# aurianer/DLA-Future

Measured on AMD Instinct MI355X. Metric: fp64 Cholesky TFlop/s, higher is better.
Workload: dtype f64; 1 GPU; cholesky_d N=65536 nb=1024 uplo=L; grid=1x1, rank_order=column-major, transport=none, work_copies=5

## Files before the change

### dla_future_amd/csrc/host/cholesky.cpp

```cpp
#include "device_matrix.hpp"
#include "launch_args.hpp"

#include <algorithm>
#include <cstdlib>
#include <cstring>
#include <vector>

namespace dlaf_mi355x {

static bool potrf_use_chain() {
  static const bool chain = [] {
    const char* e = std::getenv("DLAF_MI355X_POTRF");
    return e && std::strcmp(e, "chain") == 0;
  }();
  return chain;
}

template <class T>
void potrf_tile_coop(T* t, int ld, int kb, T* winv, int* info, int info_base, unsigned* sync, hipStream_t s,
                     bool sync_is_zero, bool count_strips) {
  launch_potrf_coop(t, ld, kb, winv, info, info_base, sync, s, sync_is_zero, count_strips);
}

template <class T>
void potrf_tile_chain(T* t, int ld, int kb, T* winv, int* info, int info_base, hipStream_t s) {
  constexpr int JB = kDiagBlock;
  for (int j0 = 0; j0 < kb; j0 += JB) {
    const int jb = std::min(JB, kb - j0);
    T* djj = t + j0 + (size_t) j0 * ld;
    T* wj = winv + (size_t) (j0 / JB) * JB * JB;
    launch_potrf_diag(djj, ld, jb, wj, info, info_base + j0, s);
    const int rem = kb - j0 - jb;
    if (rem <= 0)
      break;
    T* sub = t + (j0 + jb) + (size_t) j0 * ld;
    TrsmArgs<T> ta;
    ta.b = sub;
    ta.b_ts = 0;
    ta.ldb = ld;
    ta.il0 = 0;
    ta.il1 = 1;
    ta.pr = 1;
    ta.ri = 0;
    ta.nb = rem;
    ta.nt = 1;
    ta.last_rows = rem;
    ta.l = djj;
    ta.ldl = ld;
    ta.winv = wj;
    ta.n = jb;
    ta.info = info;
    launch_trsm(ta, s);
    UpdateArgs<T> ua;
    ua.c = t + (j0 + jb) + (size_t) (j0 + jb) * ld;
    ua.c_tsr = ua.c_tsc = 0;
    ua.ldc = ld;
    ua.a = sub;
    ua.a_ts = 0;
    ua.lda = ld;
    ua.b = sub;
    ua.b_ts = 0;
    ua.ldb = ld;
    ua.il0 = ua.jl0 = 0;
    ua.il1 = ua.jl1 = 1;
    ua.nb = rem;
    ua.K = jb;
    ua.pr = ua.pc = 1;
    ua.ri = ua.ci = 0;
    ua.nt = 1;
    ua.last_rows = rem;
    ua.info = info;
    launch_update(ua, s, 2);
  }
}

template <class T>
void potrf_tile(T* t, int ld, int kb, T* winv, int* info, int info_base, unsigned* sync, hipStream_t s) {
  if (!potrf_use_chain())
    potrf_tile_coop(t, ld, kb, winv, info, info_base, sync, s,  true,  true);
  else
    potrf_tile_chain(t, ld, kb, winv, info, info_base, s);
}

static long gcd_l(long a, long b) {
  while (b) {
    const long t = a % b;
    a = b;
    b = t;
  }
  return a;
}

template <class T>
int DeviceMatrix<T>::bcast_transposed_panel(Transport* tr, CommAxis ax_col, const T* a_base, long il_n, long jl_n,
                                            T* dst, hipStream_t s, int& period, long& ts2) {
  const size_t tile_bytes = tile_elems * sizeof(T);
  const long ncols = ltc - jl_n;
  const long g = gcd_l(rows.P, cols.P);
  period = (int) (rows.P / g);
  const long lstep = cols.P / g;
  const long cap = ncols > 0 ? (ncols + period - 1) / period : 0;
  ts2 = cap * (long) tile_elems;
  int issued = 0;
  tr->group_begin();
  for (long c = 0; c < period && c < ncols; ++c) {
    const long jl_first = jl_n + c;
    const long gj_first = cols.global_of(jl_first);
    const int root_r = rows.owner(gj_first);
    long cnt = (ncols - c + period - 1) / period;
    if (cols.global_of(jl_first + (cnt - 1) * period) == nt - 1)
      --cnt;
    if (cnt <= 0)
      continue;
    T* d = dst + c * ts2;
    if (rows.rank == root_r) {
      const T* src = a_base + (size_t) (rows.local_of(gj_first) - il_n) * tile_elems;
      DLAF_HIP_CHECK(hipMemcpy2DAsync(d, tile_bytes, src, (size_t) lstep * tile_bytes, tile_bytes, (size_t) cnt,
                                      hipMemcpyDeviceToDevice, s));
    }
    tr->bcast(ax_col, root_r, rows.rank, d, d, (size_t) cnt * tile_bytes, s);
    ++issued;
  }
  tr->group_end();
  return issued;
}

namespace {

enum class Schedule { Pairs, Sidecar, Early, Classic };

Schedule choose_schedule(bool dist, int nb, bool complex_type) {
  const char* e = std::getenv("DLAF_MI355X_SCHEDULE");
  if (e == nullptr) {
    if (dist)
      return Schedule::Early;
    if (nb % 16 == 0)
      return Schedule::Pairs;
    return !complex_type && nb <= 768 ? Schedule::Sidecar : Schedule::Classic;
  }
  if (std::strcmp(e, "early") == 0)
    return Schedule::Early;
  if (!dist && std::strcmp(e, "pairs") == 0)
    return Schedule::Pairs;
  if (!dist && std::strcmp(e, "sidecar") == 0)
    return Schedule::Sidecar;
  return Schedule::Classic;
}

constexpr long kSidecarSlots = 32;

template <class T>
struct PairRates {
  static constexpr bool dbl = sizeof(real_t<T>) == 8;
  static constexpr double r_bulk = dbl ? (TypeInfo<T>::is_complex ? 66e12 : 70e12) : 118e12;
  static constexpr double r_trsm_slot = (dbl ? 5e12 : 8e12) / 32.0;
  static constexpr double t_potrf_blk2 = 11.3e-6 * (TypeInfo<T>::is_complex ? 2.0 : 1.0);
};

template <class T>
struct Step {
  const T* a_base = nullptr;
  const T* b_base = nullptr;
  long b_ts = 0, il_n = 0, jl_n = 0;
  int b_period = 1;
  long b_ts2 = 0;
  const T* a2_base = nullptr;
  const T* b2_base = nullptr;
  int k1 = 0;
  int kb = 0;
  long rest0 = 0, split = 0;
  bool valid = false;

  static Step one_panel(int kb, long il_n, long jl_n, const T* a_base, size_t tile_elems) {
    Step st;
    st.valid = true;
    st.kb = kb;
    st.il_n = il_n;
    st.jl_n = jl_n;
    st.a_base = st.b_base = a_base;
    st.b_ts = (long) tile_elems;
    return st;
  }
  static Step two_panels(int k1, int k2, long n0, const T* a_base, const T* a2_base, size_t tile_elems) {
    Step st = one_panel(k1 + k2, n0, n0, a_base, tile_elems);
    st.k1 = k1;
    st.a2_base = st.b2_base = a2_base;
    return st;
  }
};

template <class T>
struct CholeskyIssue {
  using StepT = Step<T>;
  DeviceMatrix<T>& m;
  Transport* tr;
  const bool dist;
  const size_t tile_bytes;
  const CommAxis ax_row, ax_col;
  const hipStream_t s_main, s_panel, s_comm;
  long potrf_slots = 0, comm_slots = 0;
  long grid_reserve = 0;
  size_t next_update_slice = 0;

  explicit CholeskyIssue(DeviceMatrix<T>& mat)
      : m(mat), tr(checked_transport(*mat.grid)), dist(mat.grid->nranks > 1), tile_bytes(mat.tile_elems * sizeof(T)),
        ax_row(mat.transposed ? CommAxis::Col : CommAxis::Row),
        ax_col(mat.transposed ? CommAxis::Row : CommAxis::Col), s_main(mat.s_low), s_panel(mat.s_high),
        s_comm(mat.s_comm) {
    if (const char* e = std::getenv("DLAF_MI355X_POTRF_SLOTS"))
      potrf_slots = std::atol(e);
    else
      potrf_slots = potrf_use_chain() ? 0 : 2 * ((m.nb + kDiagBlock - 1) / kDiagBlock);
    if (const char* e = std::getenv("DLAF_MI355X_COMM_SLOTS"))
      comm_slots = std::atol(e);
    else
      comm_slots = (dist && tr->device_side()) ? 32 : 0;
    grid_reserve = potrf_slots + comm_slots;
  }

  StepT one_panel(long k, long il_n, long jl_n, const T* a_base) const {
    return StepT::one_panel(m.rows.tile_extent(k), il_n, jl_n, a_base, m.tile_elems);
  }

  void update_work(long il0, long il1, long j0, long j1, int kb, double& flops, double& bytes) const {
    flops = bytes = 0;
    const double cx = TypeInfo<T>::is_complex ? 4.0 : 1.0;
    for (long jl = j0; jl < j1; ++jl) {
      const long gj = m.cols.global_of(jl);
      const double nj = m.rows.tile_extent(gj);
      for (long il = std::max(il0, m.rows.next_local(gj)); il < il1; ++il) {
        const long gi = m.rows.global_of(il);
        const double mi = m.rows.tile_extent(gi);
        if (gi == gj) {
          flops += cx * mi * (mi + 1) * kb;
          bytes += (mi * kb + mi * mi) * sizeof(T);
        }
        else {
          flops += cx * 2.0 * mi * nj * kb;
          bytes += (mi * kb + nj * kb + 2.0 * mi * nj) * sizeof(T);
        }
      }
    }
  }

  double column_flops(const StepT& st, long jl) const {
    double f, by;
    update_work(std::max(st.il_n, m.rows.next_local(m.cols.global_of(jl))), m.ltr, jl, jl + 1, st.kb, f, by);
    return f;
  }

  void update(const StepT& st, long j0, long j1, hipStream_t s, int role, long reserve, long il_from = -1,
              long il_to = -1, int kind = -1) {
    if (!st.valid || j0 >= j1)
      return;
    const long il0 = std::max(std::max(st.il_n, il_from), m.rows.next_local(m.cols.global_of(j0)));
    const long il1 = il_to < 0 ? m.ltr : std::min(il_to, m.ltr);
    if (il0 >= il1)
      return;
    UpdateArgs<T> ua = update_args(m, il0, il1, j0, j1, st.a_base + (size_t) (il0 - st.il_n) * m.tile_elems, st.b_base,
                                   st.b_ts, st.kb, m.info);
    ua.b_period = st.b_period;
    ua.b_ts2 = st.b_ts2;
    ua.b_jl0 = (int) st.jl_n;
    if (st.k1 > 0) {
      ua.K1 = st.k1;
      ua.a2 = st.a2_base + (size_t) (il0 - st.il_n) * m.tile_elems;
      ua.b2 = st.b2_base;
    }
    double fl, by;
    update_work(il0, il1, j0, j1, st.kb, fl, by);
    const int pk = kind < 0 ? role : kind;
    m.prof_begin(pk, s);
    unsigned* cnt = m.coop_sync;
    bool zero = false;
    if (reserve > 0) {
      const size_t sl = std::min(next_update_slice, m.coop_sync_update_slices - 1);
      cnt = m.coop_sync + 16 * sl;
      zero = next_update_slice < m.coop_sync_update_slices - 1;
      ++next_update_slice;
    }
    static const bool exclusive = [] {
      const char* e = std::getenv("DLAF_MI355X_EXCLUSIVE_CUS");
      return e ? std::atoi(e) != 0 : true;
    }();
    if (reserve > 0 && exclusive)
      launch_update(ua, s, role, m.bulk_slots, cnt, zero, reserve);
    else
      launch_update(ua, s, role, reserve > 0 ? std::max<long>(8, m.bulk_slots - reserve) : 0, cnt, zero);
    DLAF_HIP_CHECK(hipGetLastError());
    m.prof_end(pk, s, fl, by);
  }

  void trsm(long il0, long il1, long klc, const T* Lkk, const T* Wkk, int kb, hipStream_t ts = nullptr) {
    if (ts == nullptr)
      ts = s_main;
    if (il0 >= il1)
      return;
    TrsmArgs<T> ta = panel_args<TrsmArgs<T>>(m, il0, il1, klc, Lkk, kb);
    ta.winv = Wkk;
    ta.info = m.info;
    ta.prio = (ts != s_main) ? 1 : 0;
    double fl = 0, by = 0;
    for (long il = il0; il < il1; ++il) {
      const double mi = m.rows.tile_extent(m.rows.global_of(il));
      fl += (TypeInfo<T>::is_complex ? 4.0 : 1.0) * (double) kb * kb * mi;
      by += (0.5 * kb * kb + 2.0 * mi * kb) * sizeof(T);
    }
    m.prof_begin(2, ts);
    launch_trsm(ta, ts);
    DLAF_HIP_CHECK(hipGetLastError());
    m.prof_end(2, ts, fl, by);
  }

  T* winv_of(long k) const { return m.winv + (size_t) (k & 1) * m.winv_elems(); }
  T* diag_ws_of(long k) const { return m.diag_ws + (size_t) (k & 1) * (m.tile_elems + m.winv_elems()); }
  void potrf(long k) {
    if (m.rows.rank != m.rows.owner(k) || m.cols.rank != m.cols.owner(k))
      return;
    const int kb = m.rows.tile_extent(k);
    const double cxf = TypeInfo<T>::is_complex ? 4.0 : 1.0;
    m.prof_begin(3, s_panel);
    potrf_tile(m.tile(m.rows.local_of(k), m.cols.local_of(k)), m.nb, kb, winv_of(k), m.info, (int) (k * m.nb),
               m.coop_sync + 16 * m.coop_sync_update_slices + m.coop_sync_potrf_words * (size_t) k, s_panel);
    DLAF_HIP_CHECK(hipGetLastError());
    m.prof_end(3, s_panel, cxf * (double) kb * kb * kb / 3.0, (double) kb * kb * sizeof(T));
  }

  void diag_bcast(long k, bool in_row, bool in_col, const T*& Lkk, const T*& Wkk) {
    Lkk = Wkk = nullptr;
    if (in_row && in_col) {
      Lkk = m.tile(m.rows.local_of(k), m.cols.local_of(k));
      Wkk = winv_of(k);
    }
    if (in_col && m.rows.P > 1) {
      T* ws = diag_ws_of(k);
      if (in_row) {
        DLAF_HIP_CHECK(hipMemcpyAsync(ws, Lkk, tile_bytes, hipMemcpyDeviceToDevice, s_panel));
        DLAF_HIP_CHECK(hipMemcpyAsync(ws + m.tile_elems, Wkk, m.winv_elems() * sizeof(T), hipMemcpyDeviceToDevice, s_panel));
      }
      DLAF_HIP_CHECK(hipEventRecord(m.ev_diag[k], s_panel));
      DLAF_HIP_CHECK(hipStreamWaitEvent(s_comm, m.ev_diag[k], 0));
      tr->bcast(ax_col, m.rows.owner(k), m.rows.rank, ws, ws, tile_bytes + m.winv_elems() * sizeof(T), s_comm);
      DLAF_HIP_CHECK(hipEventRecord(m.ev_diag[k], s_comm));
      Lkk = ws;
      Wkk = ws + m.tile_elems;
    }
    else {
      DLAF_HIP_CHECK(hipEventRecord(m.ev_diag[k], s_panel));
    }
  }

  void transposed_panel(StepT& cur, int buf) {
    if (m.rows.P > 1) {
      m.bcast_transposed_panel(tr, ax_col, cur.a_base, cur.il_n, cur.jl_n, m.panelT[buf], s_comm, cur.b_period,
                               cur.b_ts2);
      cur.b_base = m.panelT[buf];
      cur.b_ts = (long) m.tile_elems;
    }
    else {
      cur.b_base = cur.a_base + (m.cols.global_of(cur.jl_n) - cur.il_n) * (long) m.tile_elems;
      cur.b_ts = (long) m.tile_elems * m.cols.P;
    }
  }

  void join_last_diag(long k) {
    DLAF_HIP_CHECK(hipEventRecord(m.ev_diag[k], s_panel));
    DLAF_HIP_CHECK(hipStreamWaitEvent(s_main, m.ev_diag[k], 0));
  }

  void panel_done(long k, hipStream_t s) {
    DLAF_HIP_CHECK(hipEventRecord(m.ev_panel[k], s));
    m.panels_issued.store(k, std::memory_order_release);
  }

  long pair_slots(long k, double bulk_flops) const {
    using R = PairRates<T>;
    const long nb = m.nb, bulk_slots = m.bulk_slots;
    const double cxf = TypeInfo<T>::is_complex ? 4.0 : 1.0;
    const double below = (double) std::max<long>(0, m.n - (k + 1) * nb) + (double) std::max<long>(0, m.n - (k + 2) * nb);
    const double fl_t = cxf * (double) nb * nb * below;
    const double nblk = (double) nb / kDiagBlock;
    const double t_potrf = 2.0 * nblk * nblk * R::t_potrf_blk2;
    auto t_of = [&](long sl) {
      const double share = (double) sl / (double) bulk_slots;
      return std::max(bulk_flops / (R::r_bulk * (1.0 - share)), t_potrf + fl_t / (R::r_trsm_slot * (double) sl));
    };
    long best = kSidecarSlots;
    double best_t = t_of(best);
    if (bulk_flops / (R::r_bulk * (1.0 - (double) best / (double) bulk_slots)) >= best_t)
      return best;
    for (long cand : {48L, 64L, 96L, 128L, 192L, 256L}) {
      if (cand <= kSidecarSlots || cand * 2 > bulk_slots)
        continue;
      const double t = t_of(cand);
      if (t < best_t) {
        best_t = t;
        best = cand;
      }
    }
    return best;
  }

  bool u1_on_main(long k, long slots, double bulk_flops) const {
    using R = PairRates<T>;
    const long nb = m.nb;
    const double cxf = TypeInfo<T>::is_complex ? 4.0 : 1.0;
    const double below1 = (double) std::max<long>(0, m.n - (k + 1) * nb), below2 = (double) std::max<long>(0, m.n - (k + 2) * nb);
    const double fl_chain = cxf * (double) nb * nb * (below1 + below2) + cxf * 2.0 * (double) nb * nb * below1;
    const double nblk = (double) nb / kDiagBlock;
    const double t_chain = 2.0 * nblk * nblk * R::t_potrf_blk2 + fl_chain / (R::r_trsm_slot * (double) slots);
    const double t_bulk = bulk_flops / (R::r_bulk * (1.0 - (double) slots / (double) m.bulk_slots));
    return t_bulk < t_chain;
  }

  void issue_pairs();
  void issue_sidecar();
  void issue_early();
  void issue_classic();
};

template <class T>
void CholeskyIssue<T>::issue_pairs() {
  constexpr double kSplitFrac = 0.3;
  const long nt = m.nt, ltr = m.ltr, ltc = m.ltc;
  StepT prev;
  for (long k = 0; k < nt; k += 2) {
    if (tr)
      tr->mark(k);
    if (k >= 2)
      DLAF_HIP_CHECK(hipStreamWaitEvent(s_panel, m.ev_high[k - 2], 0));
    potrf(k);
    const bool second = k + 1 < nt;
    const bool more = k + 2 < nt;
    if (second) {
      trsm(k + 1, ltr, k, m.tile(k, k), winv_of(k), m.rows.tile_extent(k), s_panel);
      panel_done(k, s_panel);
    }
    const bool bulk = prev.valid && prev.rest0 < ltc;
    std::vector<double> colfl;
    double bulk_flops = 0;
    for (long jl = bulk ? prev.rest0 : ltc; jl < ltc; ++jl) {
      colfl.push_back(column_flops(prev, jl));
      bulk_flops += colfl.back();
    }
    const long slots = bulk ? pair_slots(k, bulk_flops) : kSidecarSlots;
    const bool u1_main = second && (!bulk || u1_on_main(k, slots, bulk_flops));
    long splitA = prev.rest0;
    if (u1_main && bulk) {
      double acc = 0;
      while (splitA < ltc && acc < kSplitFrac * bulk_flops)
        acc += colfl[(size_t) (splitA++ - prev.rest0)];
    }
    update(prev, prev.rest0, splitA, s_main, 0, slots);
    if (second) {
      const StepT u1 = one_panel(k, k + 1, k + 1, m.tile(k + 1 < ltr ? k + 1 : 0, k));
      if (u1_main) {
        DLAF_HIP_CHECK(hipStreamWaitEvent(s_main, m.ev_panel[k], 0));
        update(u1, k + 1, k + 2, s_main, 1, 0);
        DLAF_HIP_CHECK(hipEventRecord(m.ev_head[k], s_main));
        DLAF_HIP_CHECK(hipStreamWaitEvent(s_panel, m.ev_head[k], 0));
      }
      else {
        update(u1, k + 1, k + 2, s_panel, 1, 0);
      }
      potrf(k + 1);
      if (more) {
        trsm(k + 2, ltr, k + 1, m.tile(k + 1, k + 1), winv_of(k + 1), m.rows.tile_extent(k + 1), s_panel);
        panel_done(k + 1, s_panel);
      }
    }
    update(prev, splitA, ltc, s_main, 0, slots);
    if (!more) {
      join_last_diag(k);
      break;
    }
    DLAF_HIP_CHECK(hipStreamWaitEvent(s_main, m.ev_panel[k + 1], 0));
    StepT cur = StepT::two_panels(m.rows.tile_extent(k), m.rows.tile_extent(k + 1), k + 2, m.tile(k + 2, k),
                                  m.tile(k + 2, k + 1), m.tile_elems);
    update(cur, k + 2, std::min<long>(k + 4, ltc), s_main, 1, 0);
    DLAF_HIP_CHECK(hipEventRecord(m.ev_high[k], s_main));
    cur.rest0 = std::min<long>(k + 4, ltc);
    prev = cur;
  }
}

template <class T>
void CholeskyIssue<T>::issue_sidecar() {
  const long nt = m.nt, ltr = m.ltr, ltc = m.ltc;
  StepT prev;
  for (long k = 0; k < nt; ++k) {
    const int kb = m.rows.tile_extent(k);
    if (tr)
      tr->mark(k);
    const long il_n = m.rows.next_local(k + 1), jl_n = m.cols.next_local(k + 1);
    const long klc = m.cols.local_of(k);
    if (k >= 1)
      DLAF_HIP_CHECK(hipStreamWaitEvent(s_panel, m.ev_high[k - 1], 0));
    potrf(k);
    if (k == nt - 1) {
      update(prev, prev.rest0, ltc, s_main, 0, kSidecarSlots);
      join_last_diag(k);
      break;
    }
    trsm(il_n, ltr, klc, m.tile(m.rows.local_of(k), klc), winv_of(k), kb, s_panel);
    panel_done(k, s_panel);
    update(prev, prev.rest0, ltc, s_main, 0, kSidecarSlots);
    DLAF_HIP_CHECK(hipStreamWaitEvent(s_main, m.ev_panel[k], 0));
    StepT cur = one_panel(k, il_n, jl_n, m.tile(il_n < ltr ? il_n : 0, klc));
    transposed_panel(cur, 0);
    cur.rest0 = jl_n;
    if (jl_n < ltc) {
      update(cur, jl_n, jl_n + 1, s_main, 1, 0);
      cur.rest0 = jl_n + 1;
    }
    DLAF_HIP_CHECK(hipEventRecord(m.ev_high[k], s_main));
    prev = cur;
  }
}

template <class T>
void CholeskyIssue<T>::issue_early() {
  const long nt = m.nt, ltr = m.ltr, ltc = m.ltc;
  StepT prev;
  potrf(0);
  for (long k = 0; k < nt; ++k) {
    const int kb = m.rows.tile_extent(k);
    if (tr)
      tr->mark(k);
    const int own_c = m.cols.owner(k);
    const bool in_row = m.rows.rank == m.rows.owner(k), in_col = m.cols.rank == own_c;
    const long il_n = m.rows.next_local(k + 1), jl_n = m.cols.next_local(k + 1);
    const int buf = (int) (k & 1);
    const long klc = in_col ? m.cols.local_of(k) : -1;
    if (k == nt - 1) {
      update(prev, prev.rest0, ltc, s_main, 0, 0);
      join_last_diag(k);
      break;
    }
    const T *Lkk, *Wkk;
    diag_bcast(k, in_row, in_col, Lkk, Wkk);

    const bool head_row = m.rows.rank == m.rows.owner(k + 1);
    const long il_t = il_n + (head_row ? 1 : 0);
    DLAF_HIP_CHECK(hipStreamWaitEvent(s_main, m.ev_diag[k], 0));
    if (in_col && head_row)
      trsm(il_n, il_n + 1, klc, Lkk, Wkk, kb);
    DLAF_HIP_CHECK(hipEventRecord(m.ev_head[k], s_main));
    if (in_col)
      trsm(il_t, ltr, klc, Lkk, Wkk, kb);
    panel_done(k, s_main);

    T* dst = in_col ? m.tile(il_n < ltr ? il_n : 0, klc) : m.panel[buf];
    StepT cur = one_panel(k, il_n, jl_n, dst);
    if (dist)
      DLAF_HIP_CHECK(hipStreamWaitEvent(s_comm, m.ev_head[k], 0));
    if (m.cols.P > 1 && head_row)
      tr->bcast(ax_row, own_c, m.cols.rank, dst, dst, tile_bytes, s_comm);
    if (dist)
      DLAF_HIP_CHECK(hipEventRecord(m.ev_headb[k], s_comm));

    if (head_row && m.cols.rank == m.cols.owner(k + 1)) {
      if (k >= 1)
        DLAF_HIP_CHECK(hipStreamWaitEvent(s_panel, m.ev_high[k - 1], 0));
      DLAF_HIP_CHECK(hipStreamWaitEvent(s_panel, (dist && m.cols.P > 1) ? m.ev_headb[k] : m.ev_head[k], 0));
      update(cur, jl_n, jl_n + 1, s_panel, 2, 0, il_n, il_n + 1, 3);
      potrf(k + 1);
    }

    if (dist)
      DLAF_HIP_CHECK(hipStreamWaitEvent(s_comm, m.ev_panel[k], 0));
    if (m.cols.P > 1 && il_t < ltr)
      tr->bcast(ax_row, own_c, m.cols.rank, dst + (size_t) (il_t - il_n) * m.tile_elems,
                dst + (size_t) (il_t - il_n) * m.tile_elems, (size_t) (ltr - il_t) * tile_bytes, s_comm);
    transposed_panel(cur, buf);
    if (dist)
      DLAF_HIP_CHECK(hipEventRecord(m.ev_bcast[k], s_comm));

    update(prev, prev.rest0, ltc, s_main, 0, grid_reserve);
    if (dist)
      DLAF_HIP_CHECK(hipStreamWaitEvent(s_main, m.ev_bcast[k], 0));

    cur.rest0 = m.cols.next_local(k + 3);
    update(cur, jl_n, cur.rest0, s_main, 1, 0, m.rows.next_local(k + 2));
    DLAF_HIP_CHECK(hipEventRecord(m.ev_high[k], s_main));
    prev = cur;
  }
}

template <class T>
void CholeskyIssue<T>::issue_classic() {
  const double lookahead_flops = 270e-6 * ((double) m.nb / kDiagBlock) * 55e12;
  const long nt = m.nt, ltr = m.ltr, ltc = m.ltc;
  StepT prev;
  for (long k = 0; k < nt; ++k) {
    const int kb = m.rows.tile_extent(k);
    if (tr)
      tr->mark(k);
    const int own_c = m.cols.owner(k);
    const bool in_row = m.rows.rank == m.rows.owner(k), in_col = m.cols.rank == own_c;
    const long il_n = m.rows.next_local(k + 1), jl_n = m.cols.next_local(k + 1);
    const int buf = (int) (k & 1);
    const long klc = in_col ? m.cols.local_of(k) : -1;

    if (k >= 1)
      DLAF_HIP_CHECK(hipStreamWaitEvent(s_panel, m.ev_high[k - 1], 0));
    potrf(k);
    if (k == nt - 1) {
      update(prev, prev.rest0, prev.split, s_main, 0, potrf_slots);
      update(prev, prev.split, ltc, s_main, 0, comm_slots);
      join_last_diag(k);
      break;
    }
    const T *Lkk, *Wkk;
    diag_bcast(k, in_row, in_col, Lkk, Wkk);

    update(prev, prev.rest0, prev.split, s_main, 0, potrf_slots);

    DLAF_HIP_CHECK(hipStreamWaitEvent(s_main, m.ev_diag[k], 0));
    if (in_col)
      trsm(il_n, ltr, klc, Lkk, Wkk, kb);
    panel_done(k, s_main);

    T* dst = in_col ? m.tile(il_n < ltr ? il_n : 0, klc) : m.panel[buf];
    StepT cur = one_panel(k, il_n, jl_n, dst);
    if (dist)
      DLAF_HIP_CHECK(hipStreamWaitEvent(s_comm, m.ev_panel[k], 0));
    if (m.cols.P > 1 && il_n < ltr)
      tr->bcast(ax_row, own_c, m.cols.rank, dst, dst, (size_t) (ltr - il_n) * tile_bytes, s_comm);
    transposed_panel(cur, buf);
    if (dist)
      DLAF_HIP_CHECK(hipEventRecord(m.ev_bcast[k], s_comm));

    update(prev, prev.split, ltc, s_main, 0, comm_slots);
    if (dist)
      DLAF_HIP_CHECK(hipStreamWaitEvent(s_main, m.ev_bcast[k], 0));

    cur.rest0 = jl_n;
    if (m.cols.mine(k + 1) && jl_n < ltc) {
      update(cur, jl_n, jl_n + 1, s_main, 1, 0);
      cur.rest0 = jl_n + 1;
    }
    DLAF_HIP_CHECK(hipEventRecord(m.ev_high[k], s_main));
    cur.split = cur.rest0;
    for (double acc = 0; cur.split < ltc && acc < lookahead_flops; ++cur.split)
      acc += column_flops(cur, cur.split);
    prev = cur;
  }
}

}

template <class T>
void DeviceMatrix<T>::factorize_async() {
  CholeskyIssue<T> f(*this);
  const Schedule schedule = choose_schedule(f.dist, nb, TypeInfo<T>::is_complex);

  for (auto& ps : prof) {
    ps.used = 0;
    ps.flops = ps.bytes = ps.ms = 0;
    ps.launches = 0;
  }
  DLAF_HIP_CHECK(hipMemsetAsync(info, 0, sizeof(int), f.s_panel));
  DLAF_HIP_CHECK(hipMemsetAsync(coop_sync, 0, sizeof(unsigned) * coop_sync_words, f.s_panel));
  if (unsigned long long* tb = potrf_coop_trace_buffer())
    DLAF_HIP_CHECK(hipMemsetAsync(tb, 0, 32 * sizeof(unsigned long long), f.s_panel));
  DLAF_HIP_CHECK(hipEventRecord(ev_start[0], f.s_panel));
  DLAF_HIP_CHECK(hipStreamWaitEvent(f.s_main, ev_start[0], 0));
  DLAF_HIP_CHECK(hipStreamWaitEvent(f.s_comm, ev_start[0], 0));

  switch (schedule) {
    case Schedule::Pairs: f.issue_pairs(); break;
    case Schedule::Sidecar: f.issue_sidecar(); break;
    case Schedule::Early: f.issue_early(); break;
    case Schedule::Classic: f.issue_classic(); break;
  }

  DLAF_HIP_CHECK(hipEventRecord(ev_done[0], f.s_main));
  DLAF_HIP_CHECK(hipStreamWaitEvent(f.s_panel, ev_done[0], 0));
  DLAF_HIP_CHECK(hipMemcpyAsync(info_host, info, sizeof(int), hipMemcpyDeviceToHost, f.s_panel));
}

#define INST(T)                                                                                     \
  template void DeviceMatrix<T>::factorize_async();                                                 \
  template int DeviceMatrix<T>::bcast_transposed_panel(Transport*, CommAxis, const T*, long, long, T*, \
                                                       hipStream_t, int&, long&);                   \
  template void potrf_tile<T>(T*, int, int, T*, int*, int, unsigned*, hipStream_t);                  \
  template void potrf_tile_coop<T>(T*, int, int, T*, int*, int, unsigned*, hipStream_t, bool, bool); \
  template void potrf_tile_chain<T>(T*, int, int, T*, int*, int, hipStream_t);
INST(float)
INST(double)
INST(cfloat)
INST(cdouble)
#undef INST

}
```

Before: 71.84 TFlop/s.

## Replace pair-schedule placement heuristic with calibrated per-step cost model

Moves the pair-schedule placement decision into a new header with a richer analytical model. The model uses calibrated rates for bulk update, POTRF, TRSM and U1 under shared or exclusive CU slots. It searches over split column, slot counts for each half, and whether U1 runs on the main stream, instead of using a fixed 30% split and a single slot count. The aim is better overlap between the critical panel chain and the trailing update, but the result depends on how accurate the hard-coded rates are. An env override is added for forcing a placement.

Result: no change. 72.46 TFlop/s, median of 6 (+0.9%).

```diff
diff --git a/dla_future_amd/csrc/host/cholesky.cpp b/dla_future_amd/csrc/host/cholesky.cpp
--- a/dla_future_amd/csrc/host/cholesky.cpp
+++ b/dla_future_amd/csrc/host/cholesky.cpp
@@ -1,5 +1,6 @@
 #include "device_matrix.hpp"
 #include "launch_args.hpp"
+#include "pair_placement.hpp"
 
 #include <algorithm>
 #include <cstdlib>
@@ -150,14 +151,6 @@
 constexpr long kSidecarSlots = 32;
 
 template <class T>
-struct PairRates {
-  static constexpr bool dbl = sizeof(real_t<T>) == 8;
-  static constexpr double r_bulk = dbl ? (TypeInfo<T>::is_complex ? 66e12 : 70e12) : 118e12;
-  static constexpr double r_trsm_slot = (dbl ? 5e12 : 8e12) / 32.0;
-  static constexpr double t_potrf_blk2 = 11.3e-6 * (TypeInfo<T>::is_complex ? 2.0 : 1.0);
-};
-
-template <class T>
 struct Step {
   const T* a_base = nullptr;
   const T* b_base = nullptr;
@@ -373,46 +366,6 @@
     m.panels_issued.store(k, std::memory_order_release);
   }
 
-  long pair_slots(long k, double bulk_flops) const {
-    using R = PairRates<T>;
-    const long nb = m.nb, bulk_slots = m.bulk_slots;
-    const double cxf = TypeInfo<T>::is_complex ? 4.0 : 1.0;
-    const double below = (double) std::max<long>(0, m.n - (k + 1) * nb) + (double) std::max<long>(0, m.n - (k + 2) * nb);
-    const double fl_t = cxf * (double) nb * nb * below;
-    const double nblk = (double) nb / kDiagBlock;
-    const double t_potrf = 2.0 * nblk * nblk * R::t_potrf_blk2;
-    auto t_of = [&](long sl) {
-      const double share = (double) sl / (double) bulk_slots;
-      return std::max(bulk_flops / (R::r_bulk * (1.0 - share)), t_potrf + fl_t / (R::r_trsm_slot * (double) sl));
-    };
-    long best = kSidecarSlots;
-    double best_t = t_of(best);
-    if (bulk_flops / (R::r_bulk * (1.0 - (double) best / (double) bulk_slots)) >= best_t)
-      return best;
-    for (long cand : {48L, 64L, 96L, 128L, 192L, 256L}) {
-      if (cand <= kSidecarSlots || cand * 2 > bulk_slots)
-        continue;
-      const double t = t_of(cand);
-      if (t < best_t) {
-        best_t = t;
-        best = cand;
-      }
-    }
-    return best;
-  }
-
-  bool u1_on_main(long k, long slots, double bulk_flops) const {
-    using R = PairRates<T>;
-    const long nb = m.nb;
-    const double cxf = TypeInfo<T>::is_complex ? 4.0 : 1.0;
-    const double below1 = (double) std::max<long>(0, m.n - (k + 1) * nb), below2 = (double) std::max<long>(0, m.n - (k + 2) * nb);
-    const double fl_chain = cxf * (double) nb * nb * (below1 + below2) + cxf * 2.0 * (double) nb * nb * below1;
-    const double nblk = (double) nb / kDiagBlock;
-    const double t_chain = 2.0 * nblk * nblk * R::t_potrf_blk2 + fl_chain / (R::r_trsm_slot * (double) slots);
-    const double t_bulk = bulk_flops / (R::r_bulk * (1.0 - (double) slots / (double) m.bulk_slots));
-    return t_bulk < t_chain;
-  }
-
   void issue_pairs();
   void issue_sidecar();
   void issue_early();
@@ -421,7 +374,8 @@
 
 template <class T>
 void CholeskyIssue<T>::issue_pairs() {
-  constexpr double kSplitFrac = 0.3;
+  const PairRates rates = PairRates::of(sizeof(real_t<T>) == 8, TypeInfo<T>::is_complex);
+  const char* force = std::getenv("DLAF_MI355X_PAIR_FORCE");
   const long nt = m.nt, ltr = m.ltr, ltc = m.ltc;
   StepT prev;
   for (long k = 0; k < nt; k += 2) {
@@ -437,21 +391,23 @@
       panel_done(k, s_panel);
     }
     const bool bulk = prev.valid && prev.rest0 < ltc;
-    std::vector<double> colfl;
-    double bulk_flops = 0;
-    for (long jl = bulk ? prev.rest0 : ltc; jl < ltc; ++jl) {
-      colfl.push_back(column_flops(prev, jl));
-      bulk_flops += colfl.back();
-    }
-    const long slots = bulk ? pair_slots(k, bulk_flops) : kSidecarSlots;
-    const bool u1_main = second && (!bulk || u1_on_main(k, slots, bulk_flops));
-    long splitA = prev.rest0;
-    if (u1_main && bulk) {
-      double acc = 0;
-      while (splitA < ltc && acc < kSplitFrac * bulk_flops)
-        acc += colfl[(size_t) (splitA++ - prev.rest0)];
-    }
-    update(prev, prev.rest0, splitA, s_main, 0, slots);
+    PairGeometry geo;
+    geo.n = m.n;
+    geo.nb = m.nb;
+    geo.k = k;
+    geo.second = second;
+    geo.more = more;
+    geo.cxf = TypeInfo<T>::is_complex ? 4.0 : 1.0;
+    geo.bulk_slots = m.bulk_slots;
+    geo.rest0 = bulk ? prev.rest0 : ltc;
+    for (long jl = geo.rest0; jl < ltc; ++jl)
+      geo.colfl.push_back(column_flops(prev, jl));
+    PairPlacement pl;
+    if (!bulk || !pair_force_parse(force, geo, pl))
+      pl = place_pair(geo, rates);
+    const bool u1_main = pl.u1_main;
+    const long splitA = pl.split_col;
+    update(prev, prev.rest0, splitA, s_main, 0, pl.slots_a);
     if (second) {
       const StepT u1 = one_panel(k, k + 1, k + 1, m.tile(k + 1 < ltr ? k + 1 : 0, k));
       if (u1_main) {
@@ -469,7 +425,7 @@
         panel_done(k + 1, s_panel);
       }
     }
-    update(prev, splitA, ltc, s_main, 0, slots);
+    update(prev, splitA, ltc, s_main, 0, pl.slots_b);
     if (!more) {
       join_last_diag(k);
       break;
diff --git a/dla_future_amd/csrc/host/pair_placement.hpp b/dla_future_amd/csrc/host/pair_placement.hpp
--- /dev/null
+++ b/dla_future_amd/csrc/host/pair_placement.hpp
@@ -0,0 +1,222 @@
+#pragma once
+#include <algorithm>
+#include <cstdlib>
+#include <vector>
+
+namespace dlaf_mi355x {
+
+struct PairRates {
+  double r_bulk, r_bulk_idle, idle_share_cost, r_bulk_excl;
+  double t_potrf_beside_step, t_potrf_alone_step;
+  double r_trsm_slot, r_trsm_full, t_trsm_floor;
+  double r_u1_slot, r_u1_full;
+  double excl_slot_gain;
+  double t_drain;
+
+  static PairRates real64() {
+    return {76.0e12, 74.5e12, 0.115, 75.7e12, 67e-6, 52e-6, 0.066e12, 54e12, 0.30e-3, 0.089e12, 64e12, 1.8, 0.1e-3};
+  }
+  static PairRates complex64() {
+    return {80.8e12, 80.8e12, 1.0, 80.8e12, 130e-6, 100e-6, 0.02e12, 51e12, 0.30e-3, 0.09e12, 63e12, 6.0, 0.1e-3};
+  }
+  static PairRates real32() {
+    return {125.9e12, 125.9e12, 1.0, 125.9e12, 47e-6, 47e-6, 8e12 / 32.0, 80e12, 0.30e-3, 8e12 / 32.0, 110e12, 1.0, 0.1e-3};
+  }
+  static PairRates of(bool is_double, bool is_complex) {
+    return !is_double ? real32() : is_complex ? complex64() : real64();
+  }
+};
+
+struct PairGeometry {
+  long n = 0, nb = 0;
+  long k = 0;
+  bool second = false;
+  bool more = false;
+  double cxf = 1.0;
+  long rest0 = 0;
+  std::vector<double> colfl;
+  long bulk_slots = 0;
+  long ltc() const { return rest0 + (long) colfl.size(); }
+};
+
+struct PairPlacement {
+  long slots_a = 32, slots_b = 32;
+  bool u1_main = false;
+  long split_col = 0;
+};
+
+constexpr long kPairSlotCandidates[] = {32, 48, 64, 96, 128, 192, 256};
+constexpr long kPairSlotsDefault = 32;
+
+struct PairModel {
+  const PairGeometry& g;
+  const PairRates& r;
+  double below1, below2;
+  PairModel(const PairGeometry& geo, const PairRates& rates)
+      : g(geo), r(rates), below1((double) std::max<long>(0, geo.n - (geo.k + 1) * geo.nb)),
+        below2((double) std::max<long>(0, geo.n - (geo.k + 2) * geo.nb)) {}
+
+  static bool candidate(long slots, long bulk_slots) {
+    return slots == kPairSlotsDefault || (slots > kPairSlotsDefault && slots * 2 <= bulk_slots);
+  }
+  static bool exclusive(long slots) { return slots % 64 == 0; }
+  struct Seg {
+    double beside, alone;
+  };
+  double slot_power(long slots) const { return (double) slots * (exclusive(slots) ? r.excl_slot_gain : 1.0); }
+  Seg potrf(long slots) const {
+    const double steps = (double) g.nb / 64.0;
+    const double alone = steps * r.t_potrf_alone_step;
+    return {exclusive(slots) ? alone : steps * r.t_potrf_beside_step, alone};
+  }
+  Seg trsm(double below, long slots) const {
+    if (below <= 0)
+      return {0.0, 0.0};
+    const double fl = g.cxf * (double) g.nb * g.nb * below;
+    return {std::max(r.t_trsm_floor, fl / (r.r_trsm_slot * slot_power(slots))), std::max(r.t_trsm_floor, fl / r.r_trsm_full)};
+  }
+  double u1_flops() const { return g.cxf * 2.0 * (double) g.nb * g.nb * below1; }
+  Seg u1(long slots) const {
+    const double alone = u1_flops() / r.r_u1_full;
+    return {std::max(alone, u1_flops() / (r.r_u1_slot * slot_power(slots))), alone};
+  }
+  double u1_full() const { return u1_flops() / r.r_u1_full; }
+
+  double beside(double flops, long slots, const Seg* segs, int n) const {
+    double chain = 0, alone = 0;
+    for (int i = 0; i < n; ++i) {
+      chain += segs[i].beside;
+      alone += segs[i].alone;
+    }
+    if (flops <= 0)
+      return alone;
+    const double share = (double) slots / (double) g.bulk_slots;
+    const bool ex = exclusive(slots);
+    const double loaded = (ex ? r.r_bulk_excl : r.r_bulk) * (1.0 - share);
+    const double idle = ex ? loaded : std::max(loaded, r.r_bulk_idle * (1.0 - r.idle_share_cost * share));
+    const double t_bulk = flops / loaded;
+    if (t_bulk >= chain)
+      return chain + (flops - loaded * chain) / idle;
+    double t = t_bulk, at = 0;
+    for (int i = 0; i < n; ++i) {
+      if (at + segs[i].beside > t_bulk) {
+        const double left = segs[i].beside > 0 ? (at + segs[i].beside - std::max(at, t_bulk)) / segs[i].beside : 0.0;
+        t += left * segs[i].alone;
+      }
+      at += segs[i].beside;
+    }
+    return t;
+  }
+
+  double time_u1_slots(double bulk_flops, long slots) const {
+    Seg segs[5];
+    int n = 0;
+    segs[n++] = potrf(slots);
+    if (g.second) {
+      segs[n++] = trsm(below1, slots);
+      segs[n++] = u1(slots);
+      segs[n++] = potrf(slots);
+      segs[n++] = trsm(below2, slots);
+    }
+    return beside(bulk_flops, slots, segs, n) + r.t_drain;
+  }
+  double time_half(int half, double flops, long slots) const {
+    const Seg segs[2] = {potrf(slots), trsm(half == 0 ? below1 : below2, slots)};
+    return beside(flops, slots, segs, 2) + (flops > 0 ? r.t_drain : 0.0);
+  }
+  double time_u1_main(double flops_a, long slots_a, double flops_b, long slots_b) const {
+    return time_half(0, flops_a, slots_a) + u1_full() + r.t_drain + time_half(1, flops_b, slots_b);
+  }
+  double time(const PairPlacement& p) const {
+    double fa = 0, fb = 0;
+    for (long j = g.rest0; j < g.ltc(); ++j)
+      (j < p.split_col ? fa : fb) += g.colfl[(size_t) (j - g.rest0)];
+    if (p.u1_main)
+      return time_u1_main(fa, p.slots_a, fb, p.slots_b);
+    return time_u1_slots(fa + fb, p.slots_b) + (fa > 0 && fb > 0 ? r.t_drain : 0.0);
+  }
+};
+
+inline long best_pair_slots(const PairModel& m, int half, double flops, double* t_out = nullptr) {
+  auto t_of = [&](long s) { return half < 0 ? m.time_u1_slots(flops, s) : m.time_half(half, flops, s); };
+  long best = kPairSlotsDefault;
+  double best_t = t_of(best);
+  for (long s : kPairSlotCandidates) {
+    if (!PairModel::candidate(s, m.g.bulk_slots))
+      continue;
+    const double t = t_of(s);
+    if (t < best_t) {
+      best_t = t;
+      best = s;
+    }
+  }
+  if (t_out)
+    *t_out = best_t;
+  return best;
+}
+
+inline PairPlacement place_pair(const PairGeometry& g, const PairRates& r) {
+  PairPlacement best;
+  best.split_col = g.rest0;
+  if (g.colfl.empty()) {
+    best.u1_main = g.second;
+    return best;
+  }
+  const PairModel m(g, r);
+  double total = 0;
+  for (double f : g.colfl)
+    total += f;
+  double best_t;
+  best.slots_a = best.slots_b = best_pair_slots(m, -1, total, &best_t);
+  if (!g.second)
+    return best;
+  double fa = 0;
+  for (long cut = g.rest0; cut <= g.ltc(); ++cut) {
+    if (cut > g.rest0)
+      fa += g.colfl[(size_t) (cut - 1 - g.rest0)];
+    const double fb = cut == g.ltc() ? 0.0 : total - fa;
+    double ta, tb;
+    const long sa = best_pair_slots(m, 0, fa, &ta), sb = best_pair_slots(m, 1, fb, &tb);
+    const double t = ta + m.u1_full() + r.t_drain + tb;
+    if (t < best_t) {
+      best_t = t;
+      best.slots_a = sa;
+      best.slots_b = sb;
+      best.u1_main = true;
+      best.split_col = cut;
+    }
+  }
+  return best;
+}
+
+inline long pair_split_col(const PairGeometry& g, double frac) {
+  double total = 0, acc = 0;
+  for (double f : g.colfl)
+    total += f;
+  long col = g.rest0;
+  while (col < g.ltc() && acc < frac * total)
+    acc += g.colfl[(size_t) (col++ - g.rest0)];
+  return col;
+}
+
+inline bool pair_force_parse(const char* text, const PairGeometry& g, PairPlacement& out) {
+  if (text == nullptr)
+    return false;
+  double v[4];
+  const char* p = text;
+  for (int i = 0; i < 4; ++i) {
+    char* end = nullptr;
+    v[i] = std::strtod(p, &end);
+    if (end == p || (i < 3 && *end != ','))
+      return false;
+    p = end + 1;
+  }
+  const long hi = std::max<long>(1, g.bulk_slots - 8);
+  out.slots_a = std::min(hi, std::max<long>(1, (long) v[0]));
+  out.slots_b = std::min(hi, std::max<long>(1, (long) v[1]));
+  out.u1_main = g.second && v[2] != 0;
+  out.split_col = pair_split_col(g, std::min(1.0, std::max(0.0, v[3])));
+  return true;
+}
+
+}
```
